# thangvubk/SoftGroup

Hardware: AMD Instinct MI355X
Metric: scans/sec ScanNet-v2-like inference (softgroup_scannet.yaml, full forward_test) (higher is better)
Workload: dtype f32

## Files before the change

include/softgroup_hip.h:

```cpp
#ifndef SOFTGROUP_HIP_H
#define SOFTGROUP_HIP_H

#include <stddef.h>
#include <stdint.h>

#ifdef __cplusplus
extern "C" {
#endif

typedef void *sg_stream_t;

#define SG_OK 0
#define SG_ERR_ARG (-1)
#define SG_ERR_WORKSPACE (-2)
#define SG_ERR_LAUNCH (-3)
#define SG_ERR_UNSUPPORTED (-4)

#define SG_BALLQUERY_MAX_NEIGHBORS 1000
#define SG_OCTREE_NUM_NODES 585
#define SG_OCTREE_NUM_LEAVES 512
#define SG_LISTS_SORTED 1
#define SG_LISTS_RADIUS 2

int sg_version(void);
// ... 134 lines not shown
                            size_t ws_bytes, void *ws2, size_t ws2_bytes, sg_stream_t stream);

size_t sg_spconv_packed_weight_elems(int kvol, int cin, int cout);
int sg_spconv_pack_weight(const float *w, int cout, int kvol, int cin, int src_is_kio, float *w_k8,
                          sg_stream_t stream);

size_t sg_spconv_conv_workspace_bytes(int num_out_rows, int cout);
int sg_spconv_gather_conv_f32(const float *in, int num_in_rows, const int32_t *nbr,
                              int num_out_rows, int kvol, int cin, int cout, const float *w_k8,
                              const float *post_scale, const float *post_shift,
                              const float *residual, const float *act_scale,
                              const float *act_shift, float *out_act, const int32_t *order,
                              const uint32_t *tile_mask, const int32_t *nbr_tiles, float *out,
                              void *ws, size_t ws_bytes, sg_stream_t stream);

int sg_spconv_set_arithmetic(int mode);

int sg_spconv_set_combine(int mode);

int sg_grouping_set_lanes(int lanes);

int sg_spconv_set_chain(int mode);
int sg_spconv_chain_stats(int64_t *launches, int64_t *steps);

int sg_spconv_profile(int enable);
int sg_spconv_profile_read(double *total_ms, int *launches);
int sg_spconv_profile_detail(float *ms, int32_t *dims, int cap, int *calls);

typedef struct sg_mlp2 {
  const float *w1, *b1, *bn_scale, *bn_shift, *w2, *b2;
  int out;
} sg_mlp2;
int sg_pointwise_heads(const float *voxel_feats, const void *v2p_map, int v2p_is_int64, int n_points,
                       int channels, const sg_mlp2 *semantic, const sg_mlp2 *offset, float *output_feats,
                       float *semantic_scores, float *pt_offsets, int64_t *semantic_preds,
                       sg_stream_t stream);

size_t sg_spconv_packed_weight_elems_bf16(int kvol, int cin, int cout);
int sg_spconv_pack_weight_bf16(const float *w, int cout, int kvol, int cin, int src_is_kio,
                               uint16_t *w_k8_bf16, sg_stream_t stream);
size_t sg_spconv_conv_bf16_workspace_bytes(int num_out_rows, int cout);
int sg_spconv_gather_conv_bf16(const uint16_t *in, int num_in_rows, const int32_t *nbr, int num_out_rows,
                               int kvol, int cin, int cout, const uint16_t *w_k8_bf16,
                               const int32_t *order, const uint32_t *tile_mask, const int32_t *nbr_tiles,
                               uint16_t *out, void *ws, size_t ws_bytes, sg_stream_t stream);

// ... 549 lines not shown
```

softgroup_amd/_lib.py:

```python
import ctypes as C
import os

_HERE = os.path.dirname(os.path.abspath(__file__))
LIB_PATH = os.path.join(_HERE, 'lib', os.environ.get('SG_LIB_NAME', 'libsoftgroup_hip.so'))

_lib = None

_vp, _i, _f, _i64, _sz, _d = C.c_void_p, C.c_int, C.c_float, C.c_int64, C.c_size_t, C.c_double
_pi32 = C.POINTER(C.c_int32)

SIGNATURES = {
    'sg_version': (_i, []),
    'sg_last_error': (C.c_char_p, []),
    'sg_device_info': (_i, [C.c_char_p, _i, C.POINTER(_i), C.POINTER(_i)]),
    'sg_stream_release': (_i, [_vp]),
    'sg_host_copy_2d': (_i, [_vp, _i64, _vp, _i64, _i64, _i64]),
    'sg_host_cast_f64_f32': (_i, [_vp, _vp, _i64]),
    'sg_host_fill_i64_strided': (_i, [_vp, _i64, _i64, _i64]),
    'sg_host_colmax_i64': (_i, [_vp, _i64, _i64, _vp]),
    'sg_stream_create': (_i, [_vp]),
    'sg_stream_create_priority': (_i, [_vp, _i]),
    'sg_stream_destroy': (_i, [_vp]),
    'sg_voxelize_idx_host': (_i, [_vp, _i, _i, _i, _vp, _pi32, _pi32]),
    'sg_voxelize_idx_fill_host': (_i, [_vp, _i, _i, _i, _vp, _i, _i, _vp, _vp]),
# ... 22 lines not shown
    'sg_sec_min': (_i, [_vp, _vp, _i, _i, _vp, _vp]),
    'sg_sec_max': (_i, [_vp, _vp, _i, _i, _vp, _vp]),
    'sg_global_avg_pool_fp': (_i, [_vp, _vp, _i, _i, _vp, _vp]),
    'sg_global_avg_pool_bp': (_i, [_vp, _vp, _vp, _i, _i, _vp]),
    'sg_get_mask_iou_on_cluster': (_i, [_vp, _vp, _vp, _vp, _i, _i, _vp, _vp]),
    'sg_get_mask_iou_on_pred': (_i, [_vp, _vp, _vp, _vp, _vp, _i, _i, _vp, _vp]),
    'sg_get_mask_label': (_i, [_vp, _vp, _vp, _vp, _vp, _i, _i, _f, _vp, _vp]),
    'sg_spconv_hash_workspace_bytes': (_sz, [_i]),
    'sg_spconv_subm_rulebook': (_i, [_vp, _i, _pi32, _vp, _vp, _sz, _vp]),
    'sg_spconv_pyramid_workspace_bytes': (_sz, [_i, _i]),
    'sg_spconv_pyramid_rows': (_i, [_vp, _i, _pi32, _i, _vp, _vp, _sz, _vp]),
    'sg_spconv_pyramid_build_workspace_bytes': (_sz, [_vp, _i]),
    'sg_spconv_pyramid_build': (_i, [_vp, _i, _pi32, _i, _vp, _vp, _sz, _vp, _sz, _vp]),
    'sg_spconv_down_build': (_i, [_vp, _i, _pi32, _vp, _vp, _vp, _sz, _vp]),
    'sg_spconv_down_fill': (_i, [_vp, _i, _vp, _i, _vp, _vp, _vp, _sz, _vp]),
    'sg_spconv_inverse_rulebook': (_i, [_vp, _vp, _i, _vp, _vp]),
    'sg_spconv_plan_workspace_bytes': (_sz, [_i]),
    'sg_spconv_plan': (_i, [_vp, _i, _i, _vp, _vp, _vp, _vp, _sz, _vp]),
    'sg_spconv_set_arithmetic': (_i, [_i]),
    'sg_spconv_set_combine': (_i, [_i]),
    'sg_spconv_set_chain': (_i, [_i]),
    'sg_grouping_set_lanes': (_i, [_i]),
    'sg_spconv_chain_stats': (_i, [_vp, _vp]),
    'sg_spconv_profile': (_i, [_i]),
    'sg_spconv_profile_read': (_i, [_vp, _vp]),
    'sg_spconv_profile_detail': (_i, [_vp, _vp, _i, _vp]),
    'sg_unet_arena_bytes': (_sz, [_vp, _i]),
    'sg_unet_forward': (_i, [_vp, _vp, _vp, _i, _vp, _vp, _vp, _sz, _vp]),
    'sg_unet_train_arena_hint': (_sz, [_vp, _i]),
    'sg_unet_train_forward': (_i, [_vp, _vp, _vp, _i, _vp, _vp, _vp, _sz, _vp, _vp, _vp]),
    'sg_unet_train_backward': (_i, [_vp, _vp, _vp, _vp]),
    'sg_unet_train_release': (None, [_vp]),
    'sg_pointwise_heads': (_i, [_vp, _vp, _i, _i, _i, _vp, _vp, _vp, _vp, _vp, _vp, _vp]),
    'sg_spconv_packed_weight_elems': (_sz, [_i, _i, _i]),
    'sg_spconv_pack_weight': (_i, [_vp, _i, _i, _i, _i, _vp, _vp]),
    'sg_spconv_conv_workspace_bytes': (_sz, [_i, _i]),
    'sg_spconv_gather_conv_f32': (_i, [_vp, _i, _vp, _i, _i, _i, _i, _vp, _vp, _vp, _vp, _vp, _vp,
                                       _vp, _vp, _vp, _vp, _vp, _vp, _sz, _vp]),
    'sg_spconv_packed_weight_elems_bf16': (_sz, [_i, _i, _i]),
    'sg_spconv_pack_weight_bf16': (_i, [_vp, _i, _i, _i, _i, _vp, _vp]),
    'sg_spconv_conv_bf16_workspace_bytes': (_sz, [_i, _i]),
    'sg_spconv_gather_conv_bf16': (_i, [_vp, _i, _vp, _i, _i, _i, _i, _vp, _vp, _vp, _vp, _vp, _vp, _sz,
                                        _vp]),
    'sg_spconv_transpose_table': (_i, [_vp, _i, _i, _vp, _vp]),
    'sg_spconv_wgrad_workspace_bytes': (_sz, [_i, _i, _i, _i]),
    'sg_spconv_wgrad': (_i, [_vp, _i, _vp, _i, _vp, _i, _i, _i, _i, _vp, _vp, _sz, _vp]),
# ... 183 lines not shown
```

softgroup_amd/csrc/spconv_conv.hip:

```cpp
#include <stdlib.h>

#include <atomic>
#include <cstdio>
#include <map>
#include <mutex>
#include <utility>
#include <vector>

#include "common.h"

namespace sg {

typedef float f32x16 __attribute__((ext_vector_type(16)));
typedef float f4 __attribute__((ext_vector_type(4)));
typedef float f2 __attribute__((ext_vector_type(2)));
typedef __bf16 bf16x8 __attribute__((ext_vector_type(8)));
typedef __bf16 bf16x2 __attribute__((ext_vector_type(2)));

__device__ __forceinline__ void split3(const float (&x)[8], bf16x8 &h, bf16x8 &m, bf16x8 &l) {
#pragma unroll
  for (int j = 0; j < 4; ++j) {
    const f2 v = {x[2 * j], x[2 * j + 1]};
    const bf16x2 hh = __builtin_convertvector(v, bf16x2);
    const f2 r = v - __builtin_convertvector(hh, f2);
// ... 203 lines not shown
  }
#pragma unroll
  for (int reg = 0; reg < 16; ++reg) {
    const int r = (reg & 3) + 8 * (reg >> 2) + 4 * ahalf;
    const int row = __shfl(my_row, r, 64);
    if (row < 0) continue;
    const long long off = static_cast<long long>(row) * p.Cout + col;
#pragma unroll
    for (int n = 0; n < NBW; ++n) {
      if (n < nbw && col + n * 32 < p.Cout) {
        float v = acc[n][reg];
        if (add_res) v += p.residual[off + n * 32];
        if (post) v = fmaxf(fmaf(v, ps[n], pb[n]), 0.f);
        out[off + n * 32] = v;
        if (act) p.out_act[off + n * 32] = fmaxf(fmaf(v, as[n], ab[n]), 0.f);
      }
    }
  }
}

constexpr int kRowsAt = kTileRows * kMaxK, kMaskAt = kRowsAt + kTileRows;
constexpr int kMetaInts = kMaskAt + 4;

template <int CK, int DEPTH, int TRACE, int NBW, int SPLIT, int WV, int AT, int CHAIN, int R16 = 0>
__device__ __forceinline__ void conv_layer_body(const ConvArgs &p, unsigned in_bytes, unsigned w_bytes) {
  static_assert(!R16 || (SPLIT == 2 && AT), "bf16 rows: bf16-operand arithmetic, line-wise gather");
  constexpr int AUX = CHAIN ? 16 : 0;
  static_assert(!SPLIT || CK == 16 || AT, "split-precision path: 16-channel slices");
  static_assert(!AT || (SPLIT && CK == 32), "line-wise gather: split path, 32-channel items");
  static_assert(WV == 2 || WV == 4 || WV == 8 || WV == 16, "2, 4, 8 or 16 waves per workgroup");
  constexpr int RR = 16 / WV;
  constexpr int WV_SHIFT = WV == 2 ? 1 : WV == 4 ? 2 : WV == 8 ? 3 : 4;
  constexpr int HC = CK / 2;
  constexpr int NQ = HC / 4;
  extern __shared__ __attribute__((aligned(16))) char smem_raw[];
  const int wave = __builtin_amdgcn_readfirstlane(threadIdx.x >> 6), lane = threadIdx.x & 63;
  const int arow = lane & 31, ahalf = lane >> 5;
  float *red = reinterpret_cast<float *>(smem_raw);
  int32_t *meta_lds = reinterpret_cast<int32_t *>(red + WV * NBW * 16 * 64);

  const int G = gridDim.x;
  const int units_per_tile = p.col_units * p.ksplit;
  const int num_units = p.num_units;
  const int n_slices = R16 ? (p.Cin + 63) / 64 : p.Cin / CK;
  const int c8 = p.Cin / 8;
  const int tileK = kTileRows * p.K;
  const int nbr_base = arow * p.K;
  const bool final_out = p.ksplit == 1;
  const bool add_res = p.residual != nullptr && final_out;
  const bool post = p.post_scale != nullptr && final_out;
  const bool act = p.out_act != nullptr && final_out;
  const bool combine = p.done != nullptr && !final_out;
  const int num_tiles = (p.M_out + kTileRows - 1) / kTileRows;
  const unsigned out_bytes = static_cast<unsigned>(p.M_out) * p.Cout * 4u;
  const bool out16 = SPLIT == 2 && p.out16 != 0, res16 = SPLIT == 2 && p.res16 != 0;
  const unsigned fin_bytes = out16 ? out_bytes >> 1 : out_bytes;
  const unsigned res_bytes = res16 ? out_bytes >> 1 : out_bytes;

  const __amdgpu_buffer_rsrc_t rs_in =
      __builtin_amdgcn_make_buffer_rsrc(const_cast<float *>(p.in), 0, in_bytes, 0x00020000);
  const __amdgpu_buffer_rsrc_t rs_w =
      __builtin_amdgcn_make_buffer_rsrc(const_cast<float *>(p.w), 0, w_bytes, 0x00020000);
  const __amdgpu_buffer_rsrc_t rs_res = __builtin_amdgcn_make_buffer_rsrc(
      const_cast<float *>(add_res ? p.residual : p.in), 0, add_res ? res_bytes : 0u, 0x00020000);
  const __amdgpu_buffer_rsrc_t rs_out = __builtin_amdgcn_make_buffer_rsrc(
      p.out, 0, final_out ? fin_bytes : out_bytes * static_cast<unsigned>(p.ksplit), 0x00020000);
  const __amdgpu_buffer_rsrc_t rs_act = __builtin_amdgcn_make_buffer_rsrc(
      act ? p.out_act : p.out, 0, act ? fin_bytes : 0u, 0x00020000);
  const bool c_res = combine && p.residual != nullptr, c_act = combine && p.out_act != nullptr;
  const __amdgpu_buffer_rsrc_t rs_cres = __builtin_amdgcn_make_buffer_rsrc(
      const_cast<float *>(c_res ? p.residual : p.in), 0, c_res ? res_bytes : 0u, 0x00020000);
// ... 56 lines not shown
  };
  (void)num_tiles;

  constexpr int NPL = SPLIT == 2 ? 1 : 3;
  constexpr int NB_ = R16 ? 4 : AT ? 2 * NPL : SPLIT ? NPL : NQ;
  struct Slice { f4 a[NQ]; f4 b[NBW][NB_]; int nsl; };
  const int plane_bytes = p.K * c8 * p.Cout * 16;
  const int planes_at = 2 * plane_bytes;
  struct Ctx {
    const int32_t *meta;
    uint32_t wg_mask;
    int col, ks, k, s, kp, sp, rem;
    int pair;
    int v_w;
    float ps[NBW], pb[NBW], as[NBW], ab[NBW];
    unsigned o_off[RR];
    bool col_ok;
  };

  Slice S[DEPTH];
  float resv[NBW][RR];

  f4 *tr_lds = reinterpret_cast<f4 *>(ctl + 4) + wave * 256;
  const unsigned row_pitch = static_cast<unsigned>(p.Cin) * 4u, lane_chunk = static_cast<unsigned>(lane & 7) * 16u;
  auto load = [&](const Ctx &c, int k, int s, Slice &S) {
    if constexpr (R16) {
#pragma unroll
      for (int q = 0; q < 4; ++q) {
        const unsigned src = static_cast<unsigned>(c.meta[(8 * q + (lane >> 3)) * p.K + k]);
        const unsigned v_a = __umul24(src, row_pitch >> 1) + lane_chunk;
        S.a[q] = __builtin_bit_cast(f4, __builtin_amdgcn_raw_buffer_load_b128(rs_in, v_a, s * 128, AUX));
      }
      const int s_w = planes_at + (k * c8 + s * 8) * p.Cout * 16;
      const int nsl = s * 64 + 64 <= p.Cin ? 4 : 2;
      S.nsl = nsl;
#pragma unroll
      for (int n = 0; n < NBW; ++n)
#pragma unroll
        for (int sl = 0; sl < 4; ++sl)
          S.b[n][sl] = __builtin_bit_cast(f4, __builtin_amdgcn_raw_buffer_load_b128(
                                                  rs_w, c.v_w + n * 512, s_w + (sl < nsl ? sl : sl - 2) * (2 * p.Cout * 16), 0));
      return;
    }
    if constexpr (AT) {
#pragma unroll
      for (int q = 0; q < 4; ++q) {
        unsigned src = static_cast<unsigned>(c.meta[(8 * q + (lane >> 3)) * p.K + k]);
        if (SG_WHATIF & 16) src = static_cast<unsigned>(c.pair * 32 + 8 * q + (lane >> 3)) % static_cast<unsigned>(p.M_out);
        const unsigned v_a = __umul24(src, row_pitch) + lane_chunk;
        S.a[q] = __builtin_bit_cast(f4, __builtin_amdgcn_raw_buffer_load_b128(rs_in, v_a, s * 128, AUX));
      }
      const int s_w = planes_at + (k * c8 + s * 4) * p.Cout * 16;
#pragma unroll
      for (int n = 0; n < NBW; ++n)
#pragma unroll
        for (int sl = 0; sl < 2; ++sl)
#pragma unroll
          for (int pl = 0; pl < NPL; ++pl) {
            if ((SG_WHATIF & 1) && pl > 0) { S.b[n][sl * NPL + pl] = S.b[n][sl * NPL]; continue; }
            S.b[n][sl * NPL + pl] = __builtin_bit_cast(f4, __builtin_amdgcn_raw_buffer_load_b128(
                                                             rs_w, c.v_w + n * 512,
                                                             s_w + sl * (2 * p.Cout * 16) + pl * plane_bytes, 0));
          }
      return;
    }
    const int src = c.meta[nbr_base + k];
    const unsigned v_a = src >= 0 ? static_cast<unsigned>(src * p.Cin + ahalf * HC) * 4u : kOob;
    const int s_a = s * (CK * 4);
#pragma unroll
    for (int q = 0; q < NQ; ++q)
      S.a[q] = __builtin_bit_cast(f4, __builtin_amdgcn_raw_buffer_load_b128(rs_in, v_a + q * 16, s_a, AUX));
    if constexpr (SPLIT) {
      const int s_w = planes_at + (k * c8 + s * 2) * p.Cout * 16;
#pragma unroll
      for (int n = 0; n < NBW; ++n)
#pragma unroll
        for (int pl = 0; pl < NPL; ++pl)
          S.b[n][pl] = __builtin_bit_cast(f4, __builtin_amdgcn_raw_buffer_load_b128(
                                                  rs_w, c.v_w + n * 512, s_w + pl * plane_bytes, 0));
    } else {
      const int s_w = (k * c8 + s * (CK / 8)) * p.Cout * 32;
#pragma unroll
      for (int n = 0; n < NBW; ++n)
#pragma unroll
        for (int q = 0; q < NQ; ++q)
          S.b[n][q] = __builtin_bit_cast(f4, __builtin_amdgcn_raw_buffer_load_b128(
                                                 rs_w, c.v_w + n * 1024 + (q & 1) * 16,
                                                 s_w + (q >> 1) * (p.Cout * 32), 0));
    }
  };

  auto advance = [&](const Ctx &c, int &k, int &s) {
    if (++s == n_slices) {
      s = 0;
      const uint32_t rest = c.wg_mask & ~((2u << k) - 1u);
      k = rest ? __builtin_ctz(rest) : k;
    }
  };

  auto setup = [&](const Unit &d, int buf, Ctx &c) {
    c.ks = d.ks;
    c.pair = d.tile * p.col_units + d.cu;
    c.meta = meta_lds + buf * kMetaInts;
    uint32_t m = static_cast<uint32_t>(c.meta[kMaskAt]);
    if (!final_out) {
      const int k_lo = d.ks * p.k_per_split, k_hi = min(p.K, k_lo + p.k_per_split);
      m &= ((1u << k_hi) - 1u) & ~((1u << k_lo) - 1u);
    }
    m = __builtin_amdgcn_readfirstlane(m);
    c.wg_mask = m;
    c.col = d.cu * (32 * NBW) + arow;
    c.col_ok = c.col < p.Cout;
    const int colc = min(c.col, p.Cout - 1);
    c.v_w = SPLIT ? (ahalf * p.Cout + colc) * 16 : (ahalf * (HC / 8) * p.Cout + colc) * 32;
    const int items = __builtin_popcount(m) * n_slices;
    const int per = (items + WV - 1) >> WV_SHIFT;
    const int begin = min(items, wave * per);
    c.rem = min(items, begin + per) - begin;
    int rank = udiv(begin, p.magic_nsl);
    c.s = begin - rank * n_slices;
    uint32_t mm = m;
    for (; rank > 0; --rank) mm &= mm - 1u;
    c.k = mm ? __builtin_ctz(mm) : 0;
    load(c, c.k, c.s, S[0]);
    c.kp = c.k;
    c.sp = c.s;
#pragma unroll
    for (int i = 1; i < DEPTH - 1; ++i) {
      if (i < c.rem) advance(c, c.kp, c.sp);
      load(c, c.kp, c.sp, S[i]);
    }
    int row4[RR];
#pragma unroll
    for (int rr = 0; rr < RR; ++rr) {
      const int reg = wave * RR + rr;
      row4[rr] = c.meta[kRowsAt + (reg & 3) + 8 * (reg >> 2) + 4 * ahalf];
    }
#pragma unroll
    for (int rr = 0; rr < RR; ++rr) {
      const unsigned off = (row4[rr] >= 0 && c.col_ok)
                               ? static_cast<unsigned>(row4[rr] * p.Cout + c.col) * 4u : kOob;
      c.o_off[rr] = off;
#pragma unroll
      for (int n = 0; n < NBW; ++n)
        resv[n][rr] = ld_row(rs_res, off, n, res16);
    }
#pragma unroll
    for (int n = 0; n < NBW; ++n) {
      c.ps[n] = c.pb[n] = c.as[n] = c.ab[n] = 0.f;
      if (post) {
        c.ps[n] = p.post_scale[colc + 32 * n];
        c.pb[n] = p.post_shift[colc + 32 * n];
      }
      if (act) {
        c.as[n] = p.act_scale[colc + 32 * n];
        c.ab[n] = p.act_shift[colc + 32 * n];
      }
    }
  };

  f32x16 acc[NBW];
  auto compute = [&](Slice &S) {
    if constexpr (R16) {
#pragma unroll
      for (int q = 0; q < 4; ++q) {
        const int r = 8 * q + (lane >> 3);
        tr_lds[r * 8 + ((lane & 7) ^ ((r >> 1) & 7))] = S.a[q];
      }
      f4 fr[4];
#pragma unroll
      for (int sl = 0; sl < 4; ++sl) fr[sl] = tr_lds[arow * 8 + ((sl * 2 + ahalf) ^ ((arow >> 1) & 7))];
      const int nsl = __builtin_amdgcn_readfirstlane(S.nsl);
#pragma unroll
      for (int sl = 0; sl < 4; ++sl) {
        if (sl >= 2 && nsl == 2) break;
#pragma unroll
        for (int n = 0; n < NBW; ++n)
          acc[n] = __builtin_amdgcn_mfma_f32_32x32x16_bf16(__builtin_bit_cast(bf16x8, fr[sl]),
                                                           __builtin_bit_cast(bf16x8, S.b[n][sl]), acc[n], 0, 0, 0);
      }
      return;
    }
    if constexpr (AT) {
#pragma unroll
      for (int q = 0; q < 4; ++q) {
        const int r = 8 * q + (lane >> 3);
        if (!(SG_WHATIF & 8)) tr_lds[r * 8 + ((lane & 7) ^ ((r >> 1) & 7))] = S.a[q];
      }
      f4 fr[2][2];
#pragma unroll
      for (int sl = 0; sl < 2; ++sl)
#pragma unroll
        for (int j = 0; j < 2; ++j)
          fr[sl][j] = (SG_WHATIF & 8) ? S.a[sl * 2 + j] : tr_lds[arow * 8 + ((sl * 4 + ahalf * 2 + j) ^ ((arow >> 1) & 7))];
#pragma unroll
      for (int sl = 0; sl < 2; ++sl) {
        const float af[8] = {fr[sl][0][0], fr[sl][0][1], fr[sl][0][2], fr[sl][0][3],
                             fr[sl][1][0], fr[sl][1][1], fr[sl][1][2], fr[sl][1][3]};
        if constexpr (SPLIT == 2) {
          const bf16x8 ah = round_bf16(af);
#pragma unroll
          for (int n = 0; n < NBW; ++n)
            acc[n] = __builtin_amdgcn_mfma_f32_32x32x16_bf16(ah, __builtin_bit_cast(bf16x8, S.b[n][sl]), acc[n],
                                                             0, 0, 0);
          continue;
        }
        bf16x8 ah, am, al;
        if (SG_WHATIF & 2) {
          ah = __builtin_bit_cast(bf16x8, fr[sl][0]);
          am = __builtin_bit_cast(bf16x8, fr[sl][1]);
          al = ah;
        } else {
          split3(af, ah, am, al);
        }
#pragma unroll
        for (int n = 0; n < NBW; ++n) {
          const bf16x8 bh = __builtin_bit_cast(bf16x8, S.b[n][sl * 3 + 0]);
          const bf16x8 bm = __builtin_bit_cast(bf16x8, S.b[n][sl * 3 + 1]);
          const bf16x8 bl = __builtin_bit_cast(bf16x8, S.b[n][sl * 3 + 2]);
          if (SG_WHATIF & 4) {
            typedef int i4 __attribute__((ext_vector_type(4)));
            const i4 ax = __builtin_bit_cast(i4, al) ^ __builtin_bit_cast(i4, am) ^ __builtin_bit_cast(i4, ah);
            const i4 bx = __builtin_bit_cast(i4, bh) ^ __builtin_bit_cast(i4, bm) ^ __builtin_bit_cast(i4, bl);
            acc[n] = __builtin_amdgcn_mfma_f32_32x32x16_bf16(__builtin_bit_cast(bf16x8, ax), __builtin_bit_cast(bf16x8, bx),
                                                             acc[n], 0, 0, 0);
            continue;
          }
          acc[n] = __builtin_amdgcn_mfma_f32_32x32x16_bf16(al, bh, acc[n], 0, 0, 0);
          acc[n] = __builtin_amdgcn_mfma_f32_32x32x16_bf16(am, bm, acc[n], 0, 0, 0);
          acc[n] = __builtin_amdgcn_mfma_f32_32x32x16_bf16(ah, bl, acc[n], 0, 0, 0);
          acc[n] = __builtin_amdgcn_mfma_f32_32x32x16_bf16(am, bh, acc[n], 0, 0, 0);
          acc[n] = __builtin_amdgcn_mfma_f32_32x32x16_bf16(ah, bm, acc[n], 0, 0, 0);
          acc[n] = __builtin_amdgcn_mfma_f32_32x32x16_bf16(ah, bh, acc[n], 0, 0, 0);
        }
      }
      return;
    }
    if constexpr (SPLIT) {
      const float af[8] = {S.a[0][0], S.a[0][1], S.a[0][2], S.a[0][3], S.a[1][0], S.a[1][1], S.a[1][2], S.a[1][3]};
      if constexpr (SPLIT == 2) {
        const bf16x8 ah = round_bf16(af);
#pragma unroll
        for (int n = 0; n < NBW; ++n)
          acc[n] = __builtin_amdgcn_mfma_f32_32x32x16_bf16(ah, __builtin_bit_cast(bf16x8, S.b[n][0]), acc[n], 0,
                                                           0, 0);
        return;
      }
      bf16x8 ah, am, al;
      split3(af, ah, am, al);
#pragma unroll
      for (int n = 0; n < NBW; ++n) {
        const bf16x8 bh = __builtin_bit_cast(bf16x8, S.b[n][0]);
        const bf16x8 bm = __builtin_bit_cast(bf16x8, S.b[n][1]);
        const bf16x8 bl = __builtin_bit_cast(bf16x8, S.b[n][2]);
        acc[n] = __builtin_amdgcn_mfma_f32_32x32x16_bf16(al, bh, acc[n], 0, 0, 0);
        acc[n] = __builtin_amdgcn_mfma_f32_32x32x16_bf16(am, bm, acc[n], 0, 0, 0);
// ... 64 lines not shown
      if (un_w0 >= num_units || un_w0 < 0) {
        un_w0 = -1;
        drawing = false;
      }
      if (un_w0 >= 0) dma_meta(decode(un_w0).tile, buf ^ 1);
      if (lane == 0) ctl[buf ^ 1] = un_w0;
    }
#pragma unroll
    for (int n = 0; n < NBW; ++n)
#pragma unroll
      for (int r = 0; r < 16; ++r) acc[n][r] = 0.f;
    {
      int kp = c.kp, sp = c.sp, issued = DEPTH - 1;
      const int rem = c.rem;
      for (int g = rem / DEPTH; g > 0; --g) {
#pragma unroll
        for (int i = 0; i < DEPTH; ++i) {
          int k2 = kp, s2 = sp;
          advance(c, k2, s2);
          const bool more = issued < rem;
          kp = more ? k2 : kp;
          sp = more ? s2 : sp;
          ++issued;
          load(c, kp, sp, S[(i + DEPTH - 1) % DEPTH]);
          __builtin_amdgcn_sched_barrier(0);
          compute(S[i]);
          __builtin_amdgcn_sched_barrier(0);
        }
      }
      const int tail = rem % DEPTH;
#pragma unroll
      for (int i = 0; i < DEPTH - 1; ++i)
        if (i < tail) compute(S[i]);
    }
    if constexpr (TRACE) { asm volatile("" : "+v"(acc[0][0])); }
    mark(1);

    if (wave == 0) {
      asm volatile("s_waitcnt vmcnt(0)" ::: "memory");
      if (lane == 0 && draws)
        ticket = __hip_atomic_fetch_add(p.queue + xcd * kTicketStride, 1u, __ATOMIC_RELAXED,
                                        __HIP_MEMORY_SCOPE_AGENT);
    }

    barrier();
    mark(2);
#pragma unroll
    for (int n = 0; n < NBW; ++n)
#pragma unroll
      for (int reg = 0; reg < 16; ++reg) red[((wave * NBW + n) * 16 + reg) * 64 + lane] = acc[n][reg];
    barrier();
    mark(3);
    const int un = __builtin_amdgcn_readfirstlane(ctl[buf ^ 1]);
    const bool has_next = un >= 0;
    const Unit dn = decode(has_next ? un : u);

    float v[NBW][RR], va[NBW][RR];
    unsigned o_off[RR];
    {
      float part[NBW][RR][WV];
#pragma unroll
      for (int n = 0; n < NBW; ++n)
#pragma unroll
        for (int rr = 0; rr < RR; ++rr) {
          const int reg = wave * RR + rr;
#pragma unroll
// ... 108 lines not shown
            st_row(fmaxf(fmaf(x, as[n], ab[n]), 0.f), rs_cact, o_off[rr], 0u, n, out16);
          }
      }
    }
    mark(5);
    if constexpr (TRACE) {
      if (lane == 0 && p.trace && wave < kWavesPerWg) {
        unsigned long long *t = p.trace + (static_cast<long long>(u) * kWavesPerWg + wave) * 8;
        for (int i = 0; i < 6; ++i) t[i] = stamp[i];
        unsigned hw, xcc;
        asm volatile("s_getreg_b32 %0, hwreg(HW_REG_HW_ID)" : "=s"(hw));
        asm volatile("s_getreg_b32 %0, hwreg(HW_REG_XCC_ID)" : "=s"(xcc));
        t[6] = static_cast<unsigned long long>(blockIdx.x);
        t[7] = (static_cast<unsigned long long>(rem_done) << 48) | (static_cast<unsigned long long>(xcc & 0xf) << 32) | hw;
      }
    }
    if (!has_next) break;
    u = un;
    ++round;
    buf ^= 1;
  }
}

template <int CK, int DEPTH, int TRACE, int WPE, int NBW = 1, int SPLIT = 0, int WV = 4, int AT = 0, int R16 = 0>
__global__ void __launch_bounds__(64 * WV, WPE) gather_conv_persistent_kernel(ConvArgs p, unsigned in_bytes,
                                                                             unsigned w_bytes) {
  conv_layer_body<CK, DEPTH, TRACE, NBW, SPLIT, WV, AT, 0, R16>(p, in_bytes, w_bytes);
}

struct ChainStep {
  const float *in, *w, *post_scale, *post_shift, *residual, *act_scale, *act_shift;
  float *out_act;
  const int32_t *order;
  const uint32_t *tile_mask;
  const int32_t *nbr_tiles;
  float *out;
  unsigned *done;
  float *out_final;
  int M_out, K, Cin, Cout, col_units, ksplit, k_per_split, num_units;
  unsigned magic_upt, magic_cu, magic_nsl, in_bytes, w_bytes;
  int kind;
  int pad_[2];
};
constexpr int kChainMax = 22;
struct ChainArgs {
  ChainStep s[kChainMax];
  unsigned *bar;
  unsigned *abort_host;
  unsigned long long *trace;
  int n;
// ... 532 lines not shown
}
int conv_chain_concat(const float *a, const float *b, int64_t rows, int ca, int cb, const float *scale,
                      const float *shift, float *out, float *out_act) {
  ChainStep st = {};
  st.kind = 1;
  st.in = a; st.residual = b; st.act_scale = scale; st.act_shift = shift; st.out = out; st.out_act = out_act;
  st.M_out = static_cast<int>(rows); st.Cin = ca; st.Cout = cb;
  return chain_push(st, t_chain.b16, false);
}
int conv_chain_bn_relu(const float *x, const float *scale, const float *shift, int64_t rows, int c, float *out) {
  ChainStep st = {};
  st.kind = 2;
  st.in = x; st.post_scale = scale; st.post_shift = shift; st.out = out;
  st.M_out = static_cast<int>(rows); st.Cin = c; st.Cout = 0;
  return chain_push(st, t_chain.b16, false);
}

typedef void (*PersistentFn)(ConvArgs, unsigned, unsigned);
struct SplitVariant {
  PersistentFn fn, fn_trace;
  PersistentFn fn_b16;
  PersistentFn fn_r16;
  int nbw, wv, ck, at;
  size_t lds;
  int occ, occ_b16, occ_r16;
};
#ifndef SG_B16_DEPTH
#define SG_B16_DEPTH 2
#endif
#ifndef SG_B16_WPE_PLUS
#define SG_B16_WPE_PLUS 0
#endif
template <int CK, int WPE, int NBW, int WV, int AT>
constexpr PersistentFn r16_variant() {
  if constexpr (AT) return gather_conv_persistent_kernel<CK, SG_B16_DEPTH, 0, WPE + SG_B16_WPE_PLUS, NBW, 2, WV, 1, 1>;
  else return nullptr;
}
#define SG_SPLIT_VARIANT(CK, DEPTH, WPE, NBW, WV, AT)                                            \
  {gather_conv_persistent_kernel<CK, DEPTH, 0, WPE, NBW, 1, WV, AT>,                              \
   gather_conv_persistent_kernel<CK, DEPTH, 1, WPE, NBW, 1, WV, AT>,                              \
   gather_conv_persistent_kernel<CK, SG_B16_DEPTH, 0, WPE + SG_B16_WPE_PLUS, NBW, 2, WV, AT>,     \
   r16_variant<CK, WPE, NBW, WV, AT>(), NBW, WV, CK, AT, 0, 0, 0, 0}
constexpr int kSplitVariants = 9;
static SplitVariant g_split_variants[kSplitVariants] = {
    SG_SPLIT_VARIANT(32, 2, 2, 2, 2, 1),  SG_SPLIT_VARIANT(32, 2, 3, 1, 2, 1),
    SG_SPLIT_VARIANT(32, 2, 2, 2, 4, 1),  SG_SPLIT_VARIANT(32, 2, 3, 1, 4, 1), SG_SPLIT_VARIANT(32, 2, 1, 1, 8, 1),
    SG_SPLIT_VARIANT(16, 2, 3, 2, 4, 0),  SG_SPLIT_VARIANT(16, 2, 4, 1, 4, 0), SG_SPLIT_VARIANT(16, 2, 2, 1, 8, 0),
    SG_SPLIT_VARIANT(16, 2, 1, 1, 16, 0),
};

static int launch_persistent_split(ConvArgs a, int num_tiles, long long in_bytes, long long w_bytes,
                                   hipStream_t stream, bool b16, bool in16) {
  static int num_cu = 0;
  static std::once_flag once;
  std::call_once(once, [] {
    int dev = 0;
    hipGetDevice(&dev);
    hipDeviceGetAttribute(&num_cu, hipDeviceAttributeMultiprocessorCount, dev);
    if (num_cu <= 0) num_cu = 256;
    auto prepare = [](SplitVariant &v) {
      v.lds = static_cast<size_t>(v.wv) * v.nbw * 16 * 64 * sizeof(float) + 2 * kMetaInts * sizeof(int32_t) + 16 +
              (v.at ? static_cast<size_t>(v.wv) * 4096 : 0);
      int o = 0;
      hipOccupancyMaxActiveBlocksPerMultiprocessor(&o, v.fn, 64 * v.wv, v.lds);
      v.occ = o < 1 ? 1 : o;
      o = 0;
      hipOccupancyMaxActiveBlocksPerMultiprocessor(&o, v.fn_b16, 64 * v.wv, v.lds);
      v.occ_b16 = o < 1 ? 1 : o;
      o = 0;
      if (v.fn_r16) hipOccupancyMaxActiveBlocksPerMultiprocessor(&o, v.fn_r16, 64 * v.wv, v.lds);
      v.occ_r16 = o < 1 ? 1 : o;
    };
    for (SplitVariant &v : g_split_variants) prepare(v);
  });
  static const int nbw_env = getenv("SG_CONV_NBW") ? atoi(getenv("SG_CONV_NBW")) : 2;
  static const int wv_env = getenv("SG_CONV_WV") ? atoi(getenv("SG_CONV_WV")) : 0;
  static const float min_rounds = getenv("SG_CONV_ROUNDS") ? atof(getenv("SG_CONV_ROUNDS")) : 2.5f;
  static const int at_env = getenv("SG_CONV_AT") ? atoi(getenv("SG_CONV_AT")) : 1;
  const int NB = (a.Cout + 31) / 32;
  const unsigned long long row_bytes = (in16 ? 2ull : 4ull) * a.Cin;
  const unsigned absent_at = static_cast<unsigned>((0xFFFFFFull * row_bytes) & 0xFFFFFFFFull);
  const int use_at = ((at_env != 0 || in16) && a.Cin % 32 == 0 && in_bytes / static_cast<long long>(row_bytes) < (1LL << 24) - 1 &&
                      static_cast<long long>(absent_at) >= in_bytes) ? 1 : 0;
  if (in16 && (!use_at || !b16)) {
    set_error("sg_unet_forward(bf16 rows): a layer with %d input channels / %lld input bytes cannot take the line-wise bf16 gather",
              a.Cin, in_bytes);
    return SG_ERR_ARG;
  }
  int pick = -1;
  static const int w2_max = getenv("SG_CONV_W2_MAX") ? atoi(getenv("SG_CONV_W2_MAX")) : 108;
  static const int w2_nbw = getenv("SG_CONV_W2_NBW") ? atoi(getenv("SG_CONV_W2_NBW")) : 2;
  static const float w2_rounds = getenv("SG_CONV_W2_ROUNDS") ? atof(getenv("SG_CONV_W2_ROUNDS")) : 1.5f;
  const bool use_w2 = wv_env == 2 || (wv_env == 0 && a.K * (a.Cin / 32) <= w2_max);
  for (int i = 0; i < kSplitVariants; ++i) {
    const SplitVariant &v = g_split_variants[i];
    if (v.at != use_at) continue;
    if (v.wv == 2 && (!use_w2 || a.ksplit > 1 || v.nbw > w2_nbw)) continue;
    if (a.ksplit > 1) {
      if (v.nbw == 1 && v.wv == 4) { pick = i; break; }
      continue;
    }
    pick = i;
    if (v.nbw == 2 && (a.Cout % 64 != 0 || nbw_env < 2)) continue;
    if (wv_env && v.wv != wv_env) continue;
    const long long units = static_cast<long long>(num_tiles) * (NB / v.nbw);
    if (wv_env || units >= static_cast<long long>((v.wv == 2 ? w2_rounds : min_rounds) * num_cu * (in16 ? v.occ_r16 : b16 ? v.occ_b16 : v.occ))) {
      pick = i;
      break;
    }
  }
  const bool chain_layer = t_chain.mode != 0 && use_at != 0;
  if (chain_layer) {
    for (int i = 0; i < kSplitVariants; ++i)
      if (g_split_variants[i].at == 1 && g_split_variants[i].nbw == 1 && g_split_variants[i].wv == kChainWV) pick = i;
  }
  const SplitVariant &v = g_split_variants[pick];
  a.col_units = NB / v.nbw;
  a.blocks_per_unit = v.nbw;
  const long long units = static_cast<long long>(num_tiles) * a.col_units * a.ksplit;
  a.num_units = static_cast<int>(units);
  auto magic = [](unsigned d) { return d <= 1 ? 0u : static_cast<unsigned>((1ULL << 32) / d) + 1u; };
  a.magic_upt = magic(static_cast<unsigned>(a.col_units * a.ksplit));
  a.magic_cu = magic(static_cast<unsigned>(a.col_units));
  a.magic_nsl = magic(static_cast<unsigned>(in16 ? (a.Cin + 63) / 64 : a.Cin / v.ck));
  if (t_chain.mode == 2) {
    if (chain_layer && !in16 && !a.out16 && !a.res16 && (a.ksplit == 1 || a.done != nullptr) && stream == t_chain.stream) {
      ChainStep st = {};
      st.kind = 0;
      st.in = a.in; st.w = a.w; st.post_scale = a.post_scale; st.post_shift = a.post_shift; st.residual = a.residual;
      st.act_scale = a.act_scale; st.act_shift = a.act_shift; st.out_act = a.out_act; st.order = a.order;
      st.tile_mask = a.tile_mask; st.nbr_tiles = a.nbr_tiles; st.out = a.out; st.done = a.done; st.out_final = a.out_final;
      st.M_out = a.M_out; st.K = a.K; st.Cin = a.Cin; st.Cout = a.Cout; st.col_units = a.col_units;
      st.ksplit = a.ksplit; st.k_per_split = a.k_per_split; st.num_units = a.num_units;
      st.magic_upt = a.magic_upt; st.magic_cu = a.magic_cu; st.magic_nsl = a.magic_nsl;
      st.in_bytes = static_cast<unsigned>(in_bytes); st.w_bytes = static_cast<unsigned>(w_bytes);
      return chain_push(st, b16, a.K > 1);
    }
    const int rc = chain_flush();
    if (rc != SG_OK) return rc;
  }
  static const bool dyn_env = getenv("SG_CONV_STATIC") && atoi(getenv("SG_CONV_STATIC")) == 0;
  static const int dyn_rounds_env = getenv("SG_CONV_DYN_ROUNDS") ? atoi(getenv("SG_CONV_DYN_ROUNDS")) : 2;
  a.queue = dyn_env ? take_tickets(stream) : nullptr;
  a.dyn_rounds = dyn_rounds_env == 1 ? 1 : 2;
  long long g = static_cast<long long>(num_cu) * (in16 ? v.occ_r16 : b16 ? v.occ_b16 : v.occ);
  if (g >= 8) g -= g % 8;
  if (units < g) g = units >= 8 ? (units + 7) / 8 * 8 : units;
  const unsigned ib = static_cast<unsigned>(in_bytes), wb = static_cast<unsigned>(w_bytes);
  if (in16) {
    v.fn_r16<<<static_cast<int>(g), 64 * v.wv, v.lds, stream>>>(a, ib, wb);
    return check_launch("sg_spconv_gather_conv(bf16 rows)");
  }
  if (b16) {
    v.fn_b16<<<static_cast<int>(g), 64 * v.wv, v.lds, stream>>>(a, ib, wb);
    return check_launch("sg_spconv_gather_conv_f32(bf16 operands)");
  }
  static const char *trace_env = getenv("SG_CONV_TRACE");
  if (trace_env) {
    const size_t nb = static_cast<size_t>(units) * kWavesPerWg * 8 * sizeof(unsigned long long);
    unsigned long long *dbuf = nullptr;
    hipMalloc(&dbuf, nb);
    hipMemsetAsync(dbuf, 0, nb, stream);
    a.trace = dbuf;
    v.fn_trace<<<static_cast<int>(g), 64 * v.wv, v.lds, stream>>>(a, ib, wb);
    hipStreamSynchronize(stream);
    std::vector<unsigned long long> h(nb / 8);
    hipMemcpy(h.data(), dbuf, nb, hipMemcpyDeviceToHost);
    hipFree(dbuf);
    if (FILE *f = fopen(trace_env, "ab")) {
      long long hdr[8] = {a.M_out, a.K, a.Cin, a.Cout, units, a.col_units, v.wv, g};
      fwrite(hdr, 8, 8, f);
      fwrite(h.data(), 8, h.size(), f);
      fclose(f);
    }
  } else {
    v.fn<<<static_cast<int>(g), 64 * v.wv, v.lds, stream>>>(a, ib, wb);
  }
  return check_launch("sg_spconv_gather_conv_f32(split)");
}


}

using namespace sg;

extern "C" {

int sg_spconv_set_arithmetic(int mode) {
  SG_REQUIRE(mode >= -1 && mode <= 2, "sg_spconv_set_arithmetic: mode must be -1, 0, 1 or 2");
  g_arith_override = mode;
  return SG_OK;
}

int sg_spconv_set_combine(int mode) {
  SG_REQUIRE(mode >= -1 && mode <= 1, "sg_spconv_set_combine: mode must be -1, 0 or 1");
  g_combine_override = mode;
  return SG_OK;
}

int sg_spconv_set_chain(int mode) {
  SG_REQUIRE(mode >= -1 && mode <= 1, "sg_spconv_set_chain: mode must be -1, 0 or 1");
  g_chain_override = mode;
  return SG_OK;
}

int sg_spconv_chain_stats(int64_t *launches, int64_t *steps) {
  if (launches) *launches = g_chain_launches.load(std::memory_order_relaxed);
  if (steps) *steps = g_chain_steps.load(std::memory_order_relaxed);
  return SG_OK;
}

int sg_spconv_profile(int enable) {
  g_conv_prof.enabled = enable != 0;
  if (enable) {
    g_conv_prof.used = 0;
    g_conv_prof.dims.clear();
  }
  return SG_OK;
}

int sg_spconv_profile_detail(float *ms, int32_t *dims, int cap, int *calls) {
  const int n = static_cast<int>(g_conv_prof.used / 2);
  if (calls) *calls = n;
  for (int i = 0; i < n && i < cap; ++i) {
    if (hipEventSynchronize(g_conv_prof.pool[2 * i + 1]) != hipSuccess) {
// ... 252 lines not shown
```

Measured before the change: 436.0.

## Add lean single-buffer split-precision conv kernel variant with interleaved reloads

Adds LEAN variants of the line-wise split-precision gather-conv kernel. They drop the per-wave transpose LDS scratch by reusing the reduction buffer, and replace the two-deep slice ring with one slice whose next rows and weights are reloaded in the middle of the MFMA sequence. The epilogue loads (residual, BN scale and shift) are moved after the main loop to cut register and LDS pressure and raise occupancy. A 'wide' mode pads LDS to limit occupancy to that of the regular variant. Defaults enable lean for some wave and NBW configurations. Env knobs for forcing and grid capping, plus a query API, are added as well.

```diff
diff --git a/include/softgroup_hip.h b/include/softgroup_hip.h
--- a/include/softgroup_hip.h
+++ b/include/softgroup_hip.h
@@ -180,6 +180,8 @@
 
 int sg_spconv_set_chain(int mode);
 int sg_spconv_chain_stats(int64_t *launches, int64_t *steps);
+
+int sg_spconv_last_launch(int32_t *info);
 
 int sg_spconv_profile(int enable);
 int sg_spconv_profile_read(double *total_ms, int *launches);
diff --git a/softgroup_amd/_lib.py b/softgroup_amd/_lib.py
--- a/softgroup_amd/_lib.py
+++ b/softgroup_amd/_lib.py
@@ -68,6 +68,7 @@
     'sg_spconv_set_chain': (_i, [_i]),
     'sg_grouping_set_lanes': (_i, [_i]),
     'sg_spconv_chain_stats': (_i, [_vp, _vp]),
+    'sg_spconv_last_launch': (_i, [_vp]),
     'sg_spconv_profile': (_i, [_i]),
     'sg_spconv_profile_read': (_i, [_vp, _vp]),
     'sg_spconv_profile_detail': (_i, [_vp, _vp, _i, _vp]),
diff --git a/softgroup_amd/csrc/spconv_conv.hip b/softgroup_amd/csrc/spconv_conv.hip
--- a/softgroup_amd/csrc/spconv_conv.hip
+++ b/softgroup_amd/csrc/spconv_conv.hip
@@ -249,9 +249,11 @@
 constexpr int kRowsAt = kTileRows * kMaxK, kMaskAt = kRowsAt + kTileRows;
 constexpr int kMetaInts = kMaskAt + 4;
 
-template <int CK, int DEPTH, int TRACE, int NBW, int SPLIT, int WV, int AT, int CHAIN, int R16 = 0>
+template <int CK, int DEPTH, int TRACE, int NBW, int SPLIT, int WV, int AT, int CHAIN, int R16 = 0, int LEAN = 0>
 __device__ __forceinline__ void conv_layer_body(const ConvArgs &p, unsigned in_bytes, unsigned w_bytes) {
   static_assert(!R16 || (SPLIT == 2 && AT), "bf16 rows: bf16-operand arithmetic, line-wise gather");
+  static_assert(!LEAN || (AT && SPLIT == 1 && !R16 && !CHAIN && DEPTH == 2 && SG_WHATIF == 0),
+                "LEAN: the split-precision line-wise kernel of the single launches");
   constexpr int AUX = CHAIN ? 16 : 0;
   static_assert(!SPLIT || CK == 16 || AT, "split-precision path: 16-channel slices");
   static_assert(!AT || (SPLIT && CK == 32), "line-wise gather: split path, 32-channel items");
@@ -273,7 +275,7 @@
   const int c8 = p.Cin / 8;
   const int tileK = kTileRows * p.K;
   const int nbr_base = arow * p.K;
-  const bool final_out = p.ksplit == 1;
+  const bool final_out = LEAN || p.ksplit == 1;
   const bool add_res = p.residual != nullptr && final_out;
   const bool post = p.post_scale != nullptr && final_out;
   const bool act = p.out_act != nullptr && final_out;
@@ -376,8 +378,14 @@
   float resv[NBW][RR];
 
   f4 *tr_lds = reinterpret_cast<f4 *>(ctl + 4) + wave * 256;
+  constexpr int TR_SH = WV == 2 ? 7 : WV == 4 ? 6 : WV == 8 ? 5 : 4;
+  f4 *red4 = reinterpret_cast<f4 *>(red) + wave * RR * 16;
+  auto tr_at = [&](int t) -> f4 * {
+    if constexpr (LEAN) return red4 + (t >> TR_SH) * (NBW * 256) + (t & ((1 << TR_SH) - 1));
+    else return tr_lds + t;
+  };
   const unsigned row_pitch = static_cast<unsigned>(p.Cin) * 4u, lane_chunk = static_cast<unsigned>(lane & 7) * 16u;
-  auto load = [&](const Ctx &c, int k, int s, Slice &S) {
+  auto load = [&](const Ctx &c, int k, int s, Slice &S, bool rows_only = false) {
     if constexpr (R16) {
 #pragma unroll
       for (int q = 0; q < 4; ++q) {
@@ -404,6 +412,7 @@
         const unsigned v_a = __umul24(src, row_pitch) + lane_chunk;
         S.a[q] = __builtin_bit_cast(f4, __builtin_amdgcn_raw_buffer_load_b128(rs_in, v_a, s * 128, AUX));
       }
+      if (rows_only) return;
       const int s_w = planes_at + (k * c8 + s * 4) * p.Cout * 16;
 #pragma unroll
       for (int n = 0; n < NBW; ++n)
@@ -449,6 +458,37 @@
       s = 0;
       const uint32_t rest = c.wg_mask & ~((2u << k) - 1u);
       k = rest ? __builtin_ctz(rest) : k;
+    }
+  };
+
+  auto request_epilogue = [&](Ctx &c) {
+    const int colc = min(c.col, p.Cout - 1);
+    int row4[RR];
+#pragma unroll
+    for (int rr = 0; rr < RR; ++rr) {
+      const int reg = wave * RR + rr;
+      row4[rr] = c.meta[kRowsAt + (reg & 3) + 8 * (reg >> 2) + 4 * ahalf];
+    }
+#pragma unroll
+    for (int rr = 0; rr < RR; ++rr) {
+      const unsigned off = (row4[rr] >= 0 && c.col_ok)
+                               ? static_cast<unsigned>(row4[rr] * p.Cout + c.col) * 4u : kOob;
+      c.o_off[rr] = off;
+#pragma unroll
+      for (int n = 0; n < NBW; ++n)
+        resv[n][rr] = ld_row(rs_res, off, n, res16);
+    }
+#pragma unroll
+    for (int n = 0; n < NBW; ++n) {
+      c.ps[n] = c.pb[n] = c.as[n] = c.ab[n] = 0.f;
+      if (post) {
+        c.ps[n] = p.post_scale[colc + 32 * n];
+        c.pb[n] = p.post_shift[colc + 32 * n];
+      }
+      if (act) {
+        c.as[n] = p.act_scale[colc + 32 * n];
+        c.ab[n] = p.act_shift[colc + 32 * n];
+      }
     }
   };
 
@@ -484,37 +524,12 @@
       if (i < c.rem) advance(c, c.kp, c.sp);
       load(c, c.kp, c.sp, S[i]);
     }
-    int row4[RR];
-#pragma unroll
-    for (int rr = 0; rr < RR; ++rr) {
-      const int reg = wave * RR + rr;
-      row4[rr] = c.meta[kRowsAt + (reg & 3) + 8 * (reg >> 2) + 4 * ahalf];
-    }
-#pragma unroll
-    for (int rr = 0; rr < RR; ++rr) {
-      const unsigned off = (row4[rr] >= 0 && c.col_ok)
-                               ? static_cast<unsigned>(row4[rr] * p.Cout + c.col) * 4u : kOob;
-      c.o_off[rr] = off;
-#pragma unroll
-      for (int n = 0; n < NBW; ++n)
-        resv[n][rr] = ld_row(rs_res, off, n, res16);
-    }
-#pragma unroll
-    for (int n = 0; n < NBW; ++n) {
-      c.ps[n] = c.pb[n] = c.as[n] = c.ab[n] = 0.f;
-      if (post) {
-        c.ps[n] = p.post_scale[colc + 32 * n];
-        c.pb[n] = p.post_shift[colc + 32 * n];
-      }
-      if (act) {
-        c.as[n] = p.act_scale[colc + 32 * n];
-        c.ab[n] = p.act_shift[colc + 32 * n];
-      }
-    }
+    if constexpr (!LEAN) request_epilogue(c);
   };
 
   f32x16 acc[NBW];
-  auto compute = [&](Slice &S) {
+  auto compute = [&](Slice &S, const Ctx *cx = nullptr, int kn = 0, int sn = 0, bool reload = false) {
+    Slice &W = S;
     if constexpr (R16) {
 #pragma unroll
       for (int q = 0; q < 4; ++q) {
@@ -539,14 +554,19 @@
 #pragma unroll
       for (int q = 0; q < 4; ++q) {
         const int r = 8 * q + (lane >> 3);
-        if (!(SG_WHATIF & 8)) tr_lds[r * 8 + ((lane & 7) ^ ((r >> 1) & 7))] = S.a[q];
+        if (!(SG_WHATIF & 8)) *tr_at(r * 8 + ((lane & 7) ^ ((r >> 1) & 7))) = S.a[q];
+      }
+      const int s_wn = planes_at + (kn * c8 + sn * 4) * p.Cout * 16;
+      if constexpr (LEAN) {
+        if (reload) load(*cx, kn, sn, S, true);
+        __builtin_amdgcn_sched_barrier(0);
       }
       f4 fr[2][2];
 #pragma unroll
       for (int sl = 0; sl < 2; ++sl)
 #pragma unroll
         for (int j = 0; j < 2; ++j)
-          fr[sl][j] = (SG_WHATIF & 8) ? S.a[sl * 2 + j] : tr_lds[arow * 8 + ((sl * 4 + ahalf * 2 + j) ^ ((arow >> 1) & 7))];
+          fr[sl][j] = (SG_WHATIF & 8) ? S.a[sl * 2 + j] : *tr_at(arow * 8 + ((sl * 4 + ahalf * 2 + j) ^ ((arow >> 1) & 7)));
 #pragma unroll
       for (int sl = 0; sl < 2; ++sl) {
         const float af[8] = {fr[sl][0][0], fr[sl][0][1], fr[sl][0][2], fr[sl][0][3],
@@ -555,7 +575,7 @@
           const bf16x8 ah = round_bf16(af);
 #pragma unroll
           for (int n = 0; n < NBW; ++n)
-            acc[n] = __builtin_amdgcn_mfma_f32_32x32x16_bf16(ah, __builtin_bit_cast(bf16x8, S.b[n][sl]), acc[n],
+            acc[n] = __builtin_amdgcn_mfma_f32_32x32x16_bf16(ah, __builtin_bit_cast(bf16x8, W.b[n][sl]), acc[n],
                                                              0, 0, 0);
           continue;
         }
@@ -569,9 +589,9 @@
         }
 #pragma unroll
         for (int n = 0; n < NBW; ++n) {
-          const bf16x8 bh = __builtin_bit_cast(bf16x8, S.b[n][sl * 3 + 0]);
-          const bf16x8 bm = __builtin_bit_cast(bf16x8, S.b[n][sl * 3 + 1]);
-          const bf16x8 bl = __builtin_bit_cast(bf16x8, S.b[n][sl * 3 + 2]);
+          const bf16x8 bh = __builtin_bit_cast(bf16x8, W.b[n][sl * 3 + 0]);
+          const bf16x8 bm = __builtin_bit_cast(bf16x8, W.b[n][sl * 3 + 1]);
+          const bf16x8 bl = __builtin_bit_cast(bf16x8, W.b[n][sl * 3 + 2]);
           if (SG_WHATIF & 4) {
             typedef int i4 __attribute__((ext_vector_type(4)));
             const i4 ax = __builtin_bit_cast(i4, al) ^ __builtin_bit_cast(i4, am) ^ __builtin_bit_cast(i4, ah);
@@ -586,6 +606,16 @@
           acc[n] = __builtin_amdgcn_mfma_f32_32x32x16_bf16(am, bh, acc[n], 0, 0, 0);
           acc[n] = __builtin_amdgcn_mfma_f32_32x32x16_bf16(ah, bm, acc[n], 0, 0, 0);
           acc[n] = __builtin_amdgcn_mfma_f32_32x32x16_bf16(ah, bh, acc[n], 0, 0, 0);
+          if constexpr (LEAN) {
+            if (reload) {
+#pragma unroll
+              for (int pl = 0; pl < NPL; ++pl)
+                W.b[n][sl * NPL + pl] = __builtin_bit_cast(f4, __builtin_amdgcn_raw_buffer_load_b128(
+                                                                  rs_w, cx->v_w + n * 512,
+                                                                  s_wn + sl * (2 * p.Cout * 16) + pl * plane_bytes, 0));
+            }
+            __builtin_amdgcn_sched_barrier(0);
+          }
         }
       }
       return;
@@ -696,6 +726,11 @@
           kp = more ? k2 : kp;
           sp = more ? s2 : sp;
           ++issued;
+          if constexpr (LEAN) {
+            compute(S[0], &c, kp, sp, true);
+            __builtin_amdgcn_sched_barrier(0);
+            continue;
+          }
           load(c, kp, sp, S[(i + DEPTH - 1) % DEPTH]);
           __builtin_amdgcn_sched_barrier(0);
           compute(S[i]);
@@ -716,6 +751,8 @@
         ticket = __hip_atomic_fetch_add(p.queue + xcd * kTicketStride, 1u, __ATOMIC_RELAXED,
                                         __HIP_MEMORY_SCOPE_AGENT);
     }
+
+    if constexpr (LEAN) request_epilogue(c);
 
     barrier();
     mark(2);
@@ -870,10 +907,10 @@
   }
 }
 
-template <int CK, int DEPTH, int TRACE, int WPE, int NBW = 1, int SPLIT = 0, int WV = 4, int AT = 0, int R16 = 0>
+template <int CK, int DEPTH, int TRACE, int WPE, int NBW = 1, int SPLIT = 0, int WV = 4, int AT = 0, int R16 = 0, int LEAN = 0>
 __global__ void __launch_bounds__(64 * WV, WPE) gather_conv_persistent_kernel(ConvArgs p, unsigned in_bytes,
                                                                              unsigned w_bytes) {
-  conv_layer_body<CK, DEPTH, TRACE, NBW, SPLIT, WV, AT, 0, R16>(p, in_bytes, w_bytes);
+  conv_layer_body<CK, DEPTH, TRACE, NBW, SPLIT, WV, AT, 0, R16, LEAN>(p, in_bytes, w_bytes);
 }
 
 struct ChainStep {
@@ -1452,8 +1489,11 @@
   PersistentFn fn_b16;
   PersistentFn fn_r16;
   int nbw, wv, ck, at;
+  int lean;
   size_t lds;
   int occ, occ_b16, occ_r16;
+  size_t lds_wide;
+  int occ_wide;
 };
 #ifndef SG_B16_DEPTH
 #define SG_B16_DEPTH 2
@@ -1470,14 +1510,22 @@
   {gather_conv_persistent_kernel<CK, DEPTH, 0, WPE, NBW, 1, WV, AT>,                              \
    gather_conv_persistent_kernel<CK, DEPTH, 1, WPE, NBW, 1, WV, AT>,                              \
    gather_conv_persistent_kernel<CK, SG_B16_DEPTH, 0, WPE + SG_B16_WPE_PLUS, NBW, 2, WV, AT>,     \
-   r16_variant<CK, WPE, NBW, WV, AT>(), NBW, WV, CK, AT, 0, 0, 0, 0}
-constexpr int kSplitVariants = 9;
+   r16_variant<CK, WPE, NBW, WV, AT>(), NBW, WV, CK, AT, 0, 0, 0, 0, 0, 0, 0}
+#define SG_SPLIT_VARIANT_LEAN(CK, WPE, WPE_L, NBW, WV)                                           \
+  {gather_conv_persistent_kernel<CK, 2, 0, WPE_L, NBW, 1, WV, 1, 0, 1>,                           \
+   gather_conv_persistent_kernel<CK, 2, 1, WPE_L, NBW, 1, WV, 1, 0, 1>,                           \
+   gather_conv_persistent_kernel<CK, SG_B16_DEPTH, 0, WPE + SG_B16_WPE_PLUS, NBW, 2, WV, 1>,      \
+   r16_variant<CK, WPE, NBW, WV, 1>(), NBW, WV, CK, 1, 1, 0, 0, 0, 0, 0, 0}
+constexpr int kSplitVariants = 12;
 static SplitVariant g_split_variants[kSplitVariants] = {
     SG_SPLIT_VARIANT(32, 2, 2, 2, 2, 1),  SG_SPLIT_VARIANT(32, 2, 3, 1, 2, 1),
     SG_SPLIT_VARIANT(32, 2, 2, 2, 4, 1),  SG_SPLIT_VARIANT(32, 2, 3, 1, 4, 1), SG_SPLIT_VARIANT(32, 2, 1, 1, 8, 1),
     SG_SPLIT_VARIANT(16, 2, 3, 2, 4, 0),  SG_SPLIT_VARIANT(16, 2, 4, 1, 4, 0), SG_SPLIT_VARIANT(16, 2, 2, 1, 8, 0),
     SG_SPLIT_VARIANT(16, 2, 1, 1, 16, 0),
+    SG_SPLIT_VARIANT_LEAN(32, 2, 3, 2, 2), SG_SPLIT_VARIANT_LEAN(32, 3, 4, 1, 2), SG_SPLIT_VARIANT_LEAN(32, 3, 4, 1, 4),
 };
+
+static thread_local int t_last_split_launch[4] = {-1, -1, -1, -1};
 
 static int launch_persistent_split(ConvArgs a, int num_tiles, long long in_bytes, long long w_bytes,
                                    hipStream_t stream, bool b16, bool in16) {
@@ -1490,7 +1538,7 @@
     if (num_cu <= 0) num_cu = 256;
     auto prepare = [](SplitVariant &v) {
       v.lds = static_cast<size_t>(v.wv) * v.nbw * 16 * 64 * sizeof(float) + 2 * kMetaInts * sizeof(int32_t) + 16 +
-              (v.at ? static_cast<size_t>(v.wv) * 4096 : 0);
+              (v.at && !v.lean ? static_cast<size_t>(v.wv) * 4096 : 0);
       int o = 0;
       hipOccupancyMaxActiveBlocksPerMultiprocessor(&o, v.fn, 64 * v.wv, v.lds);
       v.occ = o < 1 ? 1 : o;
@@ -1500,6 +1548,17 @@
       o = 0;
       if (v.fn_r16) hipOccupancyMaxActiveBlocksPerMultiprocessor(&o, v.fn_r16, 64 * v.wv, v.lds);
       v.occ_r16 = o < 1 ? 1 : o;
+      v.lds_wide = v.lds;
+      v.occ_wide = v.occ;
+      if (v.lean)
+        for (const SplitVariant &pl : g_split_variants)
+          if (!pl.lean && pl.at == 1 && pl.nbw == v.nbw && pl.wv == v.wv)
+            while (v.occ_wide > pl.occ && v.lds_wide + 1024 <= 64 * 1024) {
+              v.lds_wide += 1024;
+              o = 0;
+              hipOccupancyMaxActiveBlocksPerMultiprocessor(&o, v.fn, 64 * v.wv, v.lds_wide);
+              v.occ_wide = o < 1 ? 1 : o;
+            }
     };
     for (SplitVariant &v : g_split_variants) prepare(v);
   });
@@ -1524,7 +1583,7 @@
   const bool use_w2 = wv_env == 2 || (wv_env == 0 && a.K * (a.Cin / 32) <= w2_max);
   for (int i = 0; i < kSplitVariants; ++i) {
     const SplitVariant &v = g_split_variants[i];
-    if (v.at != use_at) continue;
+    if (v.at != use_at || v.lean) continue;
     if (v.wv == 2 && (!use_w2 || a.ksplit > 1 || v.nbw > w2_nbw)) continue;
     if (a.ksplit > 1) {
       if (v.nbw == 1 && v.wv == 4) { pick = i; break; }
@@ -1539,12 +1598,33 @@
       break;
     }
   }
+  if (const char *force_env = getenv("SG_CONV_FORCE")) {
+    int f_nbw = 0, f_wv = 0;
+    if (sscanf(force_env, "%d:%d", &f_nbw, &f_wv) == 2 && use_at && a.ksplit == 1 && (f_nbw == 1 || a.Cout % 64 == 0))
+      for (int i = 0; i < kSplitVariants; ++i) {
+        const SplitVariant &v = g_split_variants[i];
+        if (v.at == 1 && !v.lean && v.nbw == f_nbw && v.wv == f_wv) pick = i;
+      }
+  }
   const bool chain_layer = t_chain.mode != 0 && use_at != 0;
   if (chain_layer) {
     for (int i = 0; i < kSplitVariants; ++i)
       if (g_split_variants[i].at == 1 && g_split_variants[i].nbw == 1 && g_split_variants[i].wv == kChainWV) pick = i;
   }
+  int lean_mode = 0;
+  if (!b16 && !in16 && !chain_layer && a.ksplit == 1 && g_split_variants[pick].at == 1) {
+    const char *lean_env = getenv("SG_CONV_LEAN");
+    const SplitVariant &o = g_split_variants[pick];
+    const int bit = o.wv == 2 ? (o.nbw == 2 ? 1 : 2) : o.wv == 4 && o.nbw == 1 ? 4 : 0;
+    const int lean_mask = lean_env ? atoi(lean_env) : bit == 1 ? (a.K > 8 ? 8 : 1) : bit == 2 ? 2 : 32;
+    lean_mode = (lean_mask & (bit << 3)) ? 2 : (lean_mask & bit) ? 1 : 0;
+    if (lean_mode)
+      for (int i = 0; i < kSplitVariants; ++i)
+        if (g_split_variants[i].lean && g_split_variants[i].nbw == o.nbw && g_split_variants[i].wv == o.wv) pick = i;
+  }
   const SplitVariant &v = g_split_variants[pick];
+  const size_t lds_fp32 = lean_mode == 2 ? v.lds_wide : v.lds;
+  const int occ_fp32 = lean_mode == 2 ? v.occ_wide : v.occ;
   a.col_units = NB / v.nbw;
   a.blocks_per_unit = v.nbw;
   const long long units = static_cast<long long>(num_tiles) * a.col_units * a.ksplit;
@@ -1573,10 +1653,16 @@
   static const int dyn_rounds_env = getenv("SG_CONV_DYN_ROUNDS") ? atoi(getenv("SG_CONV_DYN_ROUNDS")) : 2;
   a.queue = dyn_env ? take_tickets(stream) : nullptr;
   a.dyn_rounds = dyn_rounds_env == 1 ? 1 : 2;
-  long long g = static_cast<long long>(num_cu) * (in16 ? v.occ_r16 : b16 ? v.occ_b16 : v.occ);
+  long long g = static_cast<long long>(num_cu) * (in16 ? v.occ_r16 : b16 ? v.occ_b16 : occ_fp32);
   if (g >= 8) g -= g % 8;
   if (units < g) g = units >= 8 ? (units + 7) / 8 * 8 : units;
+  if (const char *cap_env = getenv("SG_CONV_GRID_MAX")) {
+    const long long cap = atoll(cap_env);
+    if (cap > 0 && g > cap) g = cap >= 8 ? cap - cap % 8 : cap;
+  }
   const unsigned ib = static_cast<unsigned>(in_bytes), wb = static_cast<unsigned>(w_bytes);
+  t_last_split_launch[0] = v.nbw; t_last_split_launch[1] = v.wv; t_last_split_launch[2] = v.lean ? lean_mode : 0;
+  t_last_split_launch[3] = static_cast<int>(g);
   if (in16) {
     v.fn_r16<<<static_cast<int>(g), 64 * v.wv, v.lds, stream>>>(a, ib, wb);
     return check_launch("sg_spconv_gather_conv(bf16 rows)");
@@ -1592,7 +1678,7 @@
     hipMalloc(&dbuf, nb);
     hipMemsetAsync(dbuf, 0, nb, stream);
     a.trace = dbuf;
-    v.fn_trace<<<static_cast<int>(g), 64 * v.wv, v.lds, stream>>>(a, ib, wb);
+    v.fn_trace<<<static_cast<int>(g), 64 * v.wv, lds_fp32, stream>>>(a, ib, wb);
     hipStreamSynchronize(stream);
     std::vector<unsigned long long> h(nb / 8);
     hipMemcpy(h.data(), dbuf, nb, hipMemcpyDeviceToHost);
@@ -1604,7 +1690,7 @@
       fclose(f);
     }
   } else {
-    v.fn<<<static_cast<int>(g), 64 * v.wv, v.lds, stream>>>(a, ib, wb);
+    v.fn<<<static_cast<int>(g), 64 * v.wv, lds_fp32, stream>>>(a, ib, wb);
   }
   return check_launch("sg_spconv_gather_conv_f32(split)");
 }
@@ -1631,6 +1717,12 @@
 int sg_spconv_set_chain(int mode) {
   SG_REQUIRE(mode >= -1 && mode <= 1, "sg_spconv_set_chain: mode must be -1, 0 or 1");
   g_chain_override = mode;
+  return SG_OK;
+}
+
+int sg_spconv_last_launch(int32_t *info) {
+  SG_REQUIRE(info != nullptr, "sg_spconv_last_launch: info is null");
+  for (int i = 0; i < 4; ++i) info[i] = t_last_split_launch[i];
   return SG_OK;
 }
 
```

Result: faster. 444.0, median of 6 (+1.8%).
